# guowentian/dynamicppr

Hardware: AMD Instinct MI355X
Metric: edge-updates/sec (ppr_throughput, summed over sources); ms_per_step = mean per-batch PPR update time (higher is better)
Workload: dtype f64

## Files before the change

### dynamicppr_amd/csrc/dppr_calib.hpp

```cpp
#pragma once

#include "dppr_common.hpp"

namespace dppr {

template <int GB>
__global__ __launch_bounds__(1024) void k_bench_lines(const double2 *__restrict__ table, uint64_t line_mask, int n_per_octet,
                                                      double *__restrict__ sink) {
    const int j = threadIdx.x & 7;
    const uint64_t oct = ((uint64_t)blockIdx.x * 1024 + threadIdx.x) >> 3;
    double a0 = 0.0, a1 = 0.0;
    for (int it = 0; it < n_per_octet; it += GB) {
        double2 v[GB];
#pragma unroll
        for (int k = 0; k < GB; ++k) {
            uint64_t z = oct * (uint64_t)n_per_octet + (uint64_t)(it + k) + 0x9E3779B97F4A7C15ull;
            z = (z ^ (z >> 30)) * 0xBF58476D1CE4E5B9ull;
            z = (z ^ (z >> 27)) * 0x94D049BB133111EBull;
            z ^= z >> 31;
            v[k] = table[(z & line_mask) * 8 + j];
        }
#pragma unroll
        for (int k = 0; k < GB; ++k) {
            a0 += v[k].x;
            a1 += v[k].y;
        }
    }
    if (a0 + a1 == 12345.678) sink[0] = a0;
}

typedef double v2d __attribute__((ext_vector_type(2)));
__global__ __launch_bounds__(1024) void k_bench_copy(const double2 *__restrict__ src2, double2 *__restrict__ dst2, int64_t n16) {
    const v2d *src = reinterpret_cast<const v2d *>(src2);
    v2d *dst = reinterpret_cast<v2d *>(dst2);
    const int64_t stride = (int64_t)gridDim.x * 1024;
    int64_t i = (int64_t)blockIdx.x * 1024 + threadIdx.x;
    for (; i + 3 * stride < n16; i += 4 * stride) {
        const v2d a = src[i], b = src[i + stride];
        const v2d c = src[i + 2 * stride], d = src[i + 3 * stride];
        dst[i] = a;
        dst[i + stride] = b;
        dst[i + 2 * stride] = c;
        dst[i + 3 * stride] = d;
    }
    for (; i < n16; i += stride) dst[i] = src[i];
}

inline int calib_device(int device) {
    int ndev = 0;
    if (hipGetDeviceCount(&ndev) != hipSuccess || device < 0 || device >= ndev) return DPPR_ERR_NO_DEVICE;
    return hipSetDevice(device) == hipSuccess ? DPPR_OK : DPPR_ERR_HIP;
}
template <class Launch>
int time_launches(int reps, float *ms_per_launch, Launch &&launch) {
    hipEvent_t a, b;
    (void)hipEventCreate(&a);
    (void)hipEventCreate(&b);
    launch();
    (void)hipEventRecord(a, 0);
    for (int i = 0; i < reps; ++i) launch();
    (void)hipEventRecord(b, 0);
// ... 11 lines not shown
```

### dynamicppr_amd/csrc/dppr_engine.hip

```cpp
#include <algorithm>
#include <atomic>
#include <cmath>
#include <cstdio>
#include <cstdlib>
#include <cstring>
#include <future>
#include <mutex>
#include <ctime>
#include <string>
#include <type_traits>
#include <unordered_map>
#include <vector>

#include <hip/hip_runtime.h>
#include <rocprim/rocprim.hpp>

#include "../../include/dppr.h"
#include "dppr_churn_plan.hpp"
#include "dppr_cut.hpp"
#include "dppr_devbuf.hpp"
#include "dppr_idspace.hpp"
#include "dppr_loop_plan.hpp"
#include "dppr_query_plan.hpp"
#include "dppr_kernels.hpp"
// ... 1612 lines not shown

int dppr_group_reset_stats(dppr_engine *e, int32_t group) {
    GET_GROUP(e, group);
    HIP_TRY(hipSetDevice(e->device));
    return solve_reset_stats(e, g);
}

int dppr_group_stats(dppr_engine *e, int32_t group, dppr_stats_t *out) {
    GET_GROUP(e, group);
    if (!out) return DPPR_ERR_INVALID;
    HIP_TRY(hipSetDevice(e->device));
    return solve_stats(e, g, out);
}

#ifdef DPPR_STAMPS
extern "C" int dppr_debug_bin_stamps(unsigned long long *out, int which, int rows) {
    return hipMemcpyFromSymbol(out, HIP_SYMBOL(dppr::g_bin_stamps), sizeof(unsigned long long) * 6 * (size_t)rows,
                               sizeof(unsigned long long) * 6 * 16384 * (size_t)which) == hipSuccess ? 0 : -2;
}
extern "C" int dppr_debug_stamps(unsigned long long *out, int rows) {
    return hipMemcpyFromSymbol(out, HIP_SYMBOL(dppr::g_stamps), sizeof(unsigned long long) * 8 * (size_t)rows) == hipSuccess
               ? 0 : -2;
}
#endif

int dppr_bench_atomics(int device, int64_t table_elems, int64_t n, int scope, int reps, float *out_ms) {
    if (table_elems <= 0 || (table_elems & (table_elems - 1)) || n <= 0 || reps <= 0 || !out_ms) return DPPR_ERR_INVALID;
    if (int rc = calib_device(device)) return rc;
    DevBuf<double> table, sink;
    if (table.alloc((size_t)table_elems) != 0) return DPPR_ERR_NOMEM;
    (void)sink.alloc(1);
    (void)hipMemset(table, 0, sizeof(double) * (size_t)table_elems);
    const int grid = 2048;
    return time_launches(reps, out_ms, [&]() {
        if (scope == 2)
            hipLaunchKernelGGL(k_bench_scatter<0>, dim3(grid), dim3(BLOCK), 0, 0, table, (uint64_t)table_elems - 1, n);
        else if (scope == 3)
            hipLaunchKernelGGL(k_bench_scatter<1>, dim3(grid), dim3(BLOCK), 0, 0, table, (uint64_t)table_elems - 1, n);
        else if (scope == 0)
            hipLaunchKernelGGL(k_bench_atomics<__HIP_MEMORY_SCOPE_AGENT>, dim3(grid), dim3(BLOCK), 0, 0, table,
                               (uint64_t)table_elems - 1, n, sink);
        else
            hipLaunchKernelGGL(k_bench_atomics<__HIP_MEMORY_SCOPE_WORKGROUP>, dim3(grid), dim3(BLOCK), 0, 0, table,
                               (uint64_t)table_elems - 1, n, sink);
    });
}

int dppr_bench_line_fills(int device, int64_t table_bytes, int64_t lines, int reps, float *out_ms) {
    if (table_bytes < 128 || (table_bytes & (table_bytes - 1)) || lines <= 0 || reps <= 0 || !out_ms) return DPPR_ERR_INVALID;
    if (int rc = calib_device(device)) return rc;
    DevBuf<double2> table;
    DevBuf<double> sink;
    if (table.alloc((size_t)table_bytes / sizeof(double2)) != 0) return DPPR_ERR_NOMEM;
    (void)sink.alloc(1);
    (void)hipMemset(table, 0, (size_t)table_bytes);
    const int grid = 2048;
    const int per = (int)std::max<int64_t>(8, (lines + (int64_t)grid * 128 - 1) / ((int64_t)grid * 128) / 8 * 8);
    const int rc = time_launches(reps, out_ms, [&]() {
        hipLaunchKernelGGL(k_bench_lines<8>, dim3(grid), dim3(1024), 0, 0, table, (uint64_t)(table_bytes / 128) - 1, per, sink);
    });
    *out_ms = *out_ms * (float)((double)lines / ((double)grid * 128.0 * per));
    return rc;
}

int dppr_bench_stream_copy(int device, int64_t bytes, int reps, float *out_ms) {
    if (bytes < 16 || reps <= 0 || !out_ms) return DPPR_ERR_INVALID;
// ... 51 lines not shown
```

### dynamicppr_amd/csrc/dppr_gpush.hpp

```cpp
#pragma once

#include "dppr_multi.hpp"

namespace dppr {

constexpr int GPUSH_LOG = 16;

struct GPushCtl {
    int n[2];
    int etot;
    int overflow;
    int it;
    int stop;
    unsigned int done;
    int pad;
    int F[GPUSH_LOG][GS_MAX];
    long long atomics[GPUSH_LOG];
};

__global__ __launch_bounds__(BLOCK) void k_gpush_list(const uint32_t *__restrict__ act, int n_words, int *__restrict__ list, int cap,
                                                      GPushCtl *__restrict__ ctl) {
    for (int w = blockIdx.x * BLOCK + threadIdx.x; w < n_words; w += gridDim.x * BLOCK) {
        uint32_t m = act[w];
        if (!m) continue;
        const int n = __popc(m);
        const int pos = atomicAdd(&ctl->n[0], n);
        for (int k = 0; m; ++k, m &= m - 1) {
            if (pos + k < cap) list[pos + k] = w * 32 + (__ffs((int)m) - 1);
            else ctl->overflow = 1;
        }
    }
}

template <int SPL, int GW>
__global__ __launch_bounds__(BLOCK) void k_gpush_rows(const int *__restrict__ list, const GPushCtl *__restrict__ ctl, int which,
                                                      double *__restrict__ x, double *__restrict__ r, bool to_x) {
    if (ctl->overflow) return;
    const int n = ctl->n[which];
    const int j = threadIdx.x & (OCT - 1);
    if (!oct_live<SPL, GW>(j)) return;
    for (int i = (blockIdx.x * BLOCK + threadIdx.x) / OCT; i < n; i += gridDim.x * BLOCK / OCT) {
        const size_t base = (size_t)list[i] * GW + j * SPL, xbase = (size_t)list[i] * x_stride(GW) + j * SPL;
#pragma unroll
        for (int q = 0; q < SPL; ++q) {
            if (to_x) x[xbase + q] = r[base + q];
            else r[base + q] = x[xbase + q];
        }
    }
}

// ... 7 lines not shown
    const int n = ctl->n[which];
    const int *list = which ? list1 : list0;
    if (threadIdx.x < GS_MAX) s_cnt[threadIdx.x] = 0;
    __syncthreads();
    const int j = threadIdx.x & (OCT - 1);
    int nleg[SPL];
#pragma unroll
    for (int q = 0; q < SPL; ++q) nleg[q] = 0;
    const bool live = oct_live<SPL, GW>(j);
    for (int i = (blockIdx.x * BLOCK + threadIdx.x) / OCT; i < n; i += gridDim.x * BLOCK / OCT) {
        const int u = list[i];
        const size_t base = (size_t)u * GW + j * SPL;
#pragma unroll
        for (int q = 0; q < SPL; ++q) {
            if (!live) continue;
            const double rv = r[base + q];
            const bool lg = legal(rv, phase, eps);
            x[(size_t)u * x_stride(GW) + j * SPL + q] = lg ? rv : 0.0;
            if (lg) {
                if (it > 0 || credit_first) p[base + q] = p[base + q] + ALPHA * rv;
                r[base + q] = 0.0;
                nleg[q]++;
            }
        }
        if (j == 0) atomicAnd(&bits[u >> 5], ~(1u << (u & 31)));
    }
#pragma unroll
    for (int q = 0; q < SPL; ++q)
        if (nleg[q]) atomicAdd(&s_cnt[j * SPL + q], nleg[q]);
    __syncthreads();
    if (threadIdx.x < GW && s_cnt[threadIdx.x]) atomicAdd(&ctl->F[it & (GPUSH_LOG - 1)][threadIdx.x], s_cnt[threadIdx.x]);
}

__global__ __launch_bounds__(1024) void k_gpush_scan(GPushCtl *ctl, const int *__restrict__ list0, const int *__restrict__ list1,
                                                     const int *__restrict__ in_row_ptr, int *__restrict__ pre, int max_n,
                                                     long long max_edges) {
    __shared__ long long s_w[16];
    __shared__ long long s_carry;
    if (ctl->stop) return;
    const int which = ctl->it & 1;
    const int n = ctl->n[which];
    const int *list = which ? list1 : list0;
    const int tid = threadIdx.x, lane = lane_id(), w = wave_id();
    if (n > max_n || ctl->overflow) {
        if (tid == 0) ctl->stop = 1;
        return;
    }
    if (tid < GS_MAX) ctl->F[ctl->it & (GPUSH_LOG - 1)][tid] = 0;
    if (tid == 0) ctl->atomics[ctl->it & (GPUSH_LOG - 1)] = 0;
    if (tid == 0) s_carry = 0;
    __syncthreads();
    for (int base = 0; base < n; base += 1024) {
        const int i = base + tid;
        int d = 0;
        if (i < n) {
            const int u = list[i];
            d = in_row_ptr[u + 1] - in_row_ptr[u];
        }
        const int inc = wave_inclusive_scan(d);
        if (lane == WAVE - 1) s_w[w] = inc;
        __syncthreads();
        long long woff = 0;
        for (int k = 0; k < w; ++k) woff += s_w[k];
        const long long carry = s_carry;
        const long long mine = carry + woff + inc - d;
        if (i < n) pre[i] = (int)(mine < 0x7fffffffll ? mine : 0x7fffffffll);
        __syncthreads();
        if (tid == 1023) s_carry = carry + woff + inc;
        __syncthreads();
    }
    if (tid == 0) {
        const long long tot = s_carry;
        if (tot > max_edges || tot > 0x7fffffffll) ctl->stop = 1;
        else {
            pre[n] = (int)tot;
            ctl->etot = (int)tot;
            ctl->n[which ^ 1] = 0;
        }
    }
}

template <int SPL, int GW>
__global__ __launch_bounds__(BLOCK) void k_gpush_expand(const int *__restrict__ list0, const int *__restrict__ list1, GPushCtl *ctl,
                                                        const int *__restrict__ pre, const int *__restrict__ in_row_ptr,
                                                        const Adj *__restrict__ adj, const int *__restrict__ hub_degp1,
                                                        const double *__restrict__ x, double *__restrict__ r,
                                                        uint32_t *__restrict__ bits, int *__restrict__ nlist0, int *__restrict__ nlist1,
                                                        int cap, int phase, double eps, IterStats *__restrict__ stats) {
    __shared__ unsigned long long s_edges;
    if (ctl->stop) return;
    const int it = ctl->it, which = it & 1;
    const int n = ctl->n[which], etot = ctl->etot;
    const int *list = which ? list1 : list0;
    int *nlist = which ? nlist0 : nlist1;
    if (threadIdx.x == 0) s_edges = 0ull;
    __syncthreads();
    const int j = threadIdx.x & (OCT - 1);
    const bool live = oct_live<SPL, GW>(j);
    const long long n_oct = (long long)gridDim.x * (BLOCK / OCT);
    const long long oct = (long long)blockIdx.x * (BLOCK / OCT) + threadIdx.x / OCT;
    const long long per = (etot + n_oct - 1) / n_oct;
    long long e0 = oct * per, e1 = e0 + per < (long long)etot ? e0 + per : (long long)etot;
    unsigned ecount = 0;
    if (e0 < e1 && n > 0) {
        int lo = 0, hi = n;
        while (hi - lo > 1) {
            const int mid = (lo + hi) >> 1;
            if (pre[mid] <= (int)e0) lo = mid; else hi = mid;
        }
        int i = lo;
        while (e0 < e1) {
            while (pre[i + 1] <= (int)e0) ++i;
            const int u = list[i];
            double xv[SPL];
#pragma unroll
            for (int q = 0; q < SPL; ++q) xv[q] = live ? x[(size_t)u * x_stride(GW) + j * SPL + q] : 0.0;
            const long long row_end = pre[i + 1] < (int)e1 ? pre[i + 1] : e1;
            const Adj *row = adj + in_row_ptr[u] + ((int)e0 - pre[i]);
            for (int k = 0; k < (int)(row_end - e0); ++k) {
                const Adj a = row[k];
                const int dp1 = a.degp1 < 0 ? hub_degp1[~a.degp1] : a.degp1;
                const double den = (double)dp1;
                bool crossed = false;
#pragma unroll
                for (int q = 0; q < SPL; ++q) {
                    if (xv[q] != 0.0) {
                        const double add = ONE_MINUS_ALPHA * xv[q] / den;
                        const double prer = atomic_add_ret(&r[(size_t)a.v * GW + j * SPL + q], add);
                        crossed |= !legal(prer, phase, eps) && legal(prer + add, phase, eps);
                        ++ecount;
                    }
                }
                if (oct_mask(__ballot(crossed)) && j == 0) {
                    const uint32_t bit = 1u << (a.v & 31);
                    const uint32_t old = atomicOr(&bits[a.v >> 5], bit);
                    if (!(old & bit)) {
                        const int pos = atomicAdd(&ctl->n[which ^ 1], 1);
                        if (pos < cap) nlist[pos] = a.v;
                        else ctl->overflow = 1;
                    }
                }
            }
            e0 = row_end;
        }
    }
    if (ecount) atomicAdd(&s_edges, (unsigned long long)ecount);
    __syncthreads();
    if (threadIdx.x == 0) {
        if (s_edges) {
            stats->blk_E[blockIdx.x] += s_edges;
            atomicAdd(reinterpret_cast<unsigned long long *>(&ctl->atomics[it & (GPUSH_LOG - 1)]), s_edges);
        }
        __threadfence();
        if (atomicAdd(&ctl->done, 1u) == gridDim.x - 1) {
            ctl->done = 0u;
            if (ctl->n[which ^ 1] > cap) ctl->n[which ^ 1] = cap;
            ctl->it = it + 1;
        }
    }
}

constexpr int TINY_N = 512;
constexpr int TINY_E = 1024;
static_assert(sizeof(double) * TINY_N * 16 + sizeof(int) * (3 * TINY_N + 1) + 1024 <= 160 * 1024,
              "k_gpush_tiny: TINY_N snapshot rows + lists + scan must fit the 160 KB LDS of a gfx950 CU");

template <int SPL, int GW>
__global__ __launch_bounds__(1024) void k_gpush_tiny(GPushCtl *ctl, int *__restrict__ list0, int *__restrict__ list1,
                                                     const int *__restrict__ in_row_ptr, const Adj *__restrict__ adj,
                                                     const int *__restrict__ hub_degp1, double *r, double *p, uint32_t *bits, int phase,
                                                     double eps, IterStats *__restrict__ stats, int max_it, int credit_first) {
    constexpr int NT = 1024, NOCT = NT / OCT;
    __shared__ int s_list[2][TINY_N];
    __shared__ int s_pre[TINY_N + 1];
    __shared__ double s_x[TINY_N * GW];
    __shared__ int s_w[NT / WAVE];
    __shared__ int s_n[2];
    __shared__ int s_cnt[GS_MAX];
    __shared__ int s_flag;
    __shared__ unsigned long long s_edges;
    if (ctl->stop || ctl->overflow) return;
    const int tid = threadIdx.x, lane = lane_id(), w = wave_id();
    const int j = tid & (OCT - 1), oid = tid / OCT;
    const bool live = oct_live<SPL, GW>(j);
    int it = ctl->it, which = it & 1;
    const int n0 = ctl->n[which];
    if (n0 > TINY_N) return;
    for (int i = tid; i < n0; i += NT) s_list[which][i] = (which ? list1 : list0)[i];
    if (tid == 0) {
        s_n[which] = n0;
        s_n[which ^ 1] = 0;
        s_flag = 0;
// ... 21 lines not shown
        if (tid < n) s_pre[tid] = woff + inc - d;
        if (tid == 0) s_pre[n] = tot;
        if (tot > TINY_E) break;
        int nleg[SPL];
#pragma unroll
        for (int q = 0; q < SPL; ++q) nleg[q] = 0;
        for (int i = oid; i < n; i += NOCT) {
            const int u = s_list[which][i];
            const size_t base = (size_t)u * GW + j * SPL;
#pragma unroll
            for (int q = 0; q < SPL; ++q) {
                if (!live) continue;
                double rv = gs_ld<true>(r + base + q);
                const bool lg = legal(rv, phase, eps);
                if (lg) {
                    rv = atomic_exch(r + base + q, 0.0);
                    if (it > 0 || credit_first) (void)__hip_atomic_fetch_add(p + base + q, ALPHA * rv, __ATOMIC_RELAXED, __HIP_MEMORY_SCOPE_AGENT);
                    nleg[q]++;
                }
                s_x[i * GW + j * SPL + q] = lg ? rv : 0.0;
            }
            if (j == 0) (void)atomicAnd(&bits[u >> 5], ~(1u << (u & 31)));
        }
#pragma unroll
        for (int q = 0; q < SPL; ++q)
            if (nleg[q]) atomicAdd(&s_cnt[j * SPL + q], nleg[q]);
        asm volatile("s_waitcnt vmcnt(0)" ::: "memory");
        __syncthreads();
        if (tid < GS_MAX) {
            ctl->F[it & (GPUSH_LOG - 1)][tid] = s_cnt[tid];
            s_cnt[tid] = 0;
        }
        const int e_per = (tot + NOCT - 1) / NOCT;
        int e0 = oid * e_per;
        const int e1 = min(tot, e0 + e_per);
        unsigned long long adds = 0;
        if (e0 < e1) {
            int lo = 0, hi = n;
            while (hi - lo > 1) {
                const int mid = (lo + hi) >> 1;
                if (s_pre[mid] <= e0) lo = mid; else hi = mid;
            }
            int i = lo;
            while (e0 < e1) {
                while (s_pre[i + 1] <= e0) ++i;
                const int u = s_list[which][i];
                double xv[SPL];
#pragma unroll
                for (int q = 0; q < SPL; ++q) xv[q] = live ? s_x[i * GW + j * SPL + q] : 0.0;
                const int row_end = min(s_pre[i + 1], e1);
                const Adj *row = adj + in_row_ptr[u] + (e0 - s_pre[i]);
                for (int k = 0; k < row_end - e0; ++k) {
                    const Adj a = row[k];
                    const double den = (double)(a.degp1 < 0 ? hub_degp1[~a.degp1] : a.degp1);
                    bool crossed = false;
#pragma unroll
                    for (int q = 0; q < SPL; ++q) {
                        if (xv[q] != 0.0) {
                            const double add = ONE_MINUS_ALPHA * xv[q] / den;
                            const double prer = atomic_add_ret(&r[(size_t)a.v * GW + j * SPL + q], add);
                            crossed |= !legal(prer, phase, eps) && legal(prer + add, phase, eps);
                            ++adds;
                        }
                    }
                    if (oct_mask(__ballot(crossed)) && j == 0) {
                        const uint32_t bit = 1u << (a.v & 31);
                        const uint32_t old = atomicOr(&bits[a.v >> 5], bit);
                        if (!(old & bit)) {
                            const int pos = atomicAdd(&s_n[which ^ 1], 1);
                            if (pos < TINY_N) s_list[which ^ 1][pos] = a.v;
                            else s_flag = 1;
                        }
                    }
                }
                e0 = row_end;
            }
        }
        if (adds) atomicAdd(&s_edges, adds);
        __syncthreads();
        if (tid == 0) {
            ctl->atomics[it & (GPUSH_LOG - 1)] = (long long)(s_edges - edges_before);
            edges_before = s_edges;
            s_n[which] = 0;
        }
        ++it;
        which ^= 1;
    }
    __syncthreads();
    const int n = min(s_n[which], TINY_N);
    for (int i = tid; i < n; i += NT) (which ? list1 : list0)[i] = s_list[which][i];
    if (tid == 0) {
        ctl->n[which] = n;
        ctl->n[which ^ 1] = 0;
        ctl->it = it;
        if (s_flag) ctl->stop = 1;
        if (s_edges) stats->blk_E[0] += s_edges;
    }
}

template <int SPL, int GW>
__global__ __launch_bounds__(BLOCK) void k_gpush_leave(int V, const uint32_t *__restrict__ bits, double *__restrict__ x,
                                                       const double *__restrict__ r, double *__restrict__ p, int credit, int phase,
                                                       double eps, int *__restrict__ cnt_out) {
    __shared__ int s_cnt[GS_MAX];
    if (threadIdx.x < GS_MAX) s_cnt[threadIdx.x] = 0;
    __syncthreads();
    const int j = threadIdx.x & (OCT - 1);
    const bool live = oct_live<SPL, GW>(j);
    int nleg[SPL];
#pragma unroll
// ... 23 lines not shown
```

### dynamicppr_amd/csrc/dppr_host_group.hpp

```cpp
#pragma once

namespace {

template <class F>
void with_row(int gw, int nvx, F &&f) {
    auto narrow = [&](auto w) {
        if (nvx == 512) f(IC<1>{}, w, IC<512>{});
        else f(IC<1>{}, w, IC<1024>{});
    };
    switch (gw) {
    case 2: narrow(IC<2>{}); break;
    case 4: narrow(IC<4>{}); break;
    case 6: narrow(IC<6>{}); break;
    case 8: narrow(IC<8>{}); break;
    case 10: f(IC<2>{}, IC<10>{}, IC<512>{}); break;
    case 12: f(IC<2>{}, IC<12>{}, IC<512>{}); break;
    case 14: f(IC<2>{}, IC<14>{}, IC<512>{}); break;
    default: f(IC<2>{}, IC<16>{}, IC<512>{}); break;
    }
}
template <class F>
void with_row(int gw, F &&f) {
    with_row(gw, 512, [&](auto spl, auto w, auto) { f(spl, w); });
}
// ... 36 lines not shown
        cap = std::min(per_cu * cus, STAT_SLOTS);
    }
    return cap;
}

struct PushTail {
    enum How { NOT_ENTERED, CONVERGED, GAVE_BACK } how = NOT_ENTERED;
    int iters = 0;
    bool owed = false;
};

int group_push_tail(dppr_engine *e, Group &g, const Epoch &ep, int phase, double eps, long long pairs_at_entry, PushTail *t) {
    const int cap = std::max(1024, std::min(e->gpush_list_cap, e->V));
    if (g.plist[0].capacity() != (size_t)cap || !g.pctl) {
        HIP_TRY(loop_wait(e));
        g.plist[0].reset(); g.plist[1].reset(); g.ppre.reset(); g.pctl.reset();
        HIP_TRY(g.plist[0].alloc((size_t)cap));
        HIP_TRY(g.plist[1].alloc((size_t)cap));
        HIP_TRY(g.ppre.alloc((size_t)cap + 1));
        HIP_TRY(g.pctl.alloc(1));
    }
    HIP_TRY(hipMemsetAsync(g.pctl, 0, sizeof(GPushCtl), e->stream));
    const int n_words = (ep.grp_n_int + 31) / 32;
    hipLaunchKernelGGL(k_gpush_list, dim3(grid_for(n_words)), dim3(BLOCK), 0, e->stream, g.act[0], n_words, g.plist[0], cap, g.pctl);
    const int rows_grid = grid_for(std::min<long long>(pairs_at_entry, cap), BLOCK / OCT);
    with_row(g.gw, [&](auto spl, auto gw) {
        hipLaunchKernelGGL((k_gpush_rows<decltype(spl)::value, decltype(gw)::value>), dim3(rows_grid), dim3(BLOCK), 0, e->stream, g.plist[0],
                           g.pctl, 0, g.x, g.r, false);
    });
    HIP_TRY(hipGetLastError());
    static thread_local GPushCtl h;
    const int credit_first = t->owed ? 1 : 0;
    const long long max_edges = gpush_edge_bound(e->gpush_max_edges, ep.n_ggroups);
    const int grid = 256;
    static const bool trace = getenv("DPPR_GROUP_TRACE") != nullptr;
    int it_done = 0;
    long long known_n = pairs_at_entry;
    bool tiny_declined = false;
    long long last_adds = gpush_adds_at_entry(pairs_at_entry);
    for (;;) {
        if (gpush_take_tiny(known_n, last_adds, tiny_declined)) {
            with_row(g.gw, [&](auto spl, auto gw) {
                hipLaunchKernelGGL((k_gpush_tiny<decltype(spl)::value, decltype(gw)::value>), dim3(1), dim3(1024), 0, e->stream, g.pctl, g.plist[0],
                                   g.plist[1], ep.row_ptr, ep.adj, ep.hub_degp1, g.r, g.p, g.act[0], phase, eps, g.dstats, GPUSH_LOG, credit_first);
            });
        } else {
        const int m = gpush_chunk(it_done, pairs_at_entry);
        tiny_declined = false;
        for (int k = 0; k < m; ++k) {
            hipLaunchKernelGGL(k_gpush_scan, dim3(1), dim3(1024), 0, e->stream, g.pctl, g.plist[0], g.plist[1], ep.row_ptr, g.ppre, cap - 1, max_edges);
            with_row(g.gw, [&](auto spl, auto gw) {
                constexpr int SPL = decltype(spl)::value, GW = decltype(gw)::value;
                hipLaunchKernelGGL((k_gpush_snap<SPL, GW>), dim3(grid), dim3(BLOCK), 0, e->stream, g.plist[0], g.plist[1], g.pctl, g.x, g.r, g.p,
                                   g.act[0], phase, eps, credit_first);
                hipLaunchKernelGGL((k_gpush_expand<SPL, GW>), dim3(grid), dim3(BLOCK), 0, e->stream, g.plist[0], g.plist[1], g.pctl, g.ppre,
                                   ep.row_ptr, ep.adj, ep.hub_degp1, g.x, g.r, g.act[0], g.plist[0], g.plist[1], cap, phase, eps, g.dstats);
            });
        }
        }
        HIP_TRY(hipGetLastError());
        HIP_TRY(hipMemcpyAsync(&h, g.pctl, sizeof(GPushCtl), hipMemcpyDeviceToHost, e->stream));
        HIP_TRY(loop_wait(e));
        for (int i = it_done; i < h.it; ++i) {
            const long long F = lane_sum(h.F[i & (GPUSH_LOG - 1)]);
            if (F == 0) continue;
            account_iteration(g.st, F, ITER_PUSH);
            ++t->iters;
            if (trace)
                fprintf(stderr, "[gpush ] phase %d iteration +%d  frontier pairs %9lld  adds %lld\n", phase, i, F, h.atomics[i & (GPUSH_LOG - 1)]);
        }
        if (gpush_tiny_declined(h.it > it_done, h.stop != 0, known_n)) tiny_declined = true;
        if (h.it > it_done) last_adds = h.atomics[(h.it - 1) & (GPUSH_LOG - 1)];
        it_done = h.it;
        known_n = h.n[h.it & 1];
        if (h.stop && h.it == 0 && h.overflow) return DPPR_OK;
        if (h.stop) {
            if (trace) fprintf(stderr, "[gpush ] phase %d: an iteration of %d vertices called itself off after %d iterations\n", phase, h.n[h.it & 1], h.it);
            HIP_TRY(hipMemsetAsync(g.cnt, 0, sizeof(int) * 3 * GS_MAX, e->stream));
            with_row(g.gw, [&](auto spl, auto gw) {
                hipLaunchKernelGGL((k_gpush_leave<decltype(spl)::value, decltype(gw)::value>), dim3(grid_for(ep.grp_n_int, BLOCK / OCT)), dim3(BLOCK), 0,
                                   e->stream, ep.grp_n_int, g.act[0], g.x, g.r, g.p, h.it > 0 ? 1 : 0, phase, eps, g.cnt);
            });
            HIP_TRY(hipGetLastError());
            if (h.it > 0) t->owed = false;
            t->how = PushTail::GAVE_BACK;
            return DPPR_OK;
        }
        if (h.n[h.it & 1] == 0) {
            t->how = PushTail::CONVERGED;
            return DPPR_OK;
        }
        if (it_done >= e->max_iters) return fail(e, DPPR_ERR_NOT_CONVERGED, "iteration cap hit");
    }
}

struct GroupLoop {
    dppr_engine *const e;
    Group &g;
    const Epoch &ep;
    const int phase;
    const double eps;
    const int hp = phase == PHASE_BOTH ? 0 : phase;
// ... 183 lines not shown
```

### dynamicppr_amd/csrc/dppr_host_state.hpp

```cpp
#pragma once

static constexpr int CNT_HDR = 16;
static constexpr int PERSIST_RETRY_BATCHES = 64;
static constexpr int GQ_PAD = 32;
static constexpr int BIN_MAX_BLOCKS = 1 << 16, BIN_MAX_BIG = 4096, BIN_SMALL_INTS = BIN_MAX_BLOCKS + BIN_MAX_BIG + 1 + 64;
static constexpr int SU_SPLIT_MIN = 1 << 16;
static constexpr int MERGE_MISS_WORD = 44;

namespace dppr {

inline std::atomic<long long> g_device_bytes{0}, g_pinned_bytes{0};

struct DeviceAlloc {
    static int alloc(void **p, size_t bytes) {
        const hipError_t rc = hipMalloc(p, bytes);
        if (rc == hipSuccess) g_device_bytes.fetch_add((long long)bytes, std::memory_order_relaxed);
        return (int)rc;
    }
    static int free(void *p, size_t bytes) {
        g_device_bytes.fetch_sub((long long)bytes, std::memory_order_relaxed);
        return (int)hipFree(p);
    }
};

// ... 265 lines not shown
    size_t sort_tmp_bytes = 0;
    DevBuf<int> su_grp;
    DevBuf<uint64_t> bk[4];
    DevBuf<uint64_t> bks[4];
    DevBuf<int> delpos;
    struct Pre {
        std::future<bool> task;
        const int32_t *src[4] = {nullptr, nullptr, nullptr, nullptr};
        int n[4] = {0, 0, 0, 0};
        std::vector<int32_t> out[4];
        std::vector<uint32_t> miss[4];
        unsigned long long epoch = 0;
        bool armed = false, ok = false;
    } pre;
    long long pre_hits = 0, pre_misses = 0;
    bool incremental = true;
    bool sweep_bits = false;
    bool hot_blocks = true;
    int gsweep_hot_rows = 24576;
    int gsweep_grid_cap = 0;
    bool group_resident = true;
    int gmulti_cap[2] = {-1, -1};
    bool any_groups = false;
    int ggroups_min = 256;
    bool force_radix_grouping = false;
    bool cost_model = true;
    bool group_full_rows = false;
    bool wide_groups = false;
    bool group_tail_seeding = true;
    int gpush_enter_pairs = -1;
    int gpush_list_cap = 1 << 20;
    long long gpush_max_edges = 0;
    int gpush_auto_factor = 2;
    int bin_mode = 1;
    int bin_ha_tiles = 128, bin_hb_tiles = 60;
    long long bin_target = 0;
    long long bin_target_a = 4ll << 20;
    long long bin_min_ids = 1ll << 19;
    DevBuf<int> bin_vblk_a;
    DevBuf<unsigned long long> bin_scan;
    DevBuf<int> bin_small;
    long long bin_chunk = 32768;
    DevBuf<double> bin_vals;
    DevBuf<uint64_t> bin_wb, bin_wa;
    DevBuf<int> bin_first;
    std::vector<int32_t> bin_cut_a, bin_cut_b;
    int bin_abits = 0, bin_bbits = 0;
    int bin_cut_ids = 0;
    bool bin_words_valid = false;
    int bin_slides_since_cut = 0;
    bool bin_incremental = true;
    int bin_recut_every = 32;
    bool bin_frozen_rebuild = false;
    bool bin_force_full = false;
    int bin_miss_host = 0;
    long long bin_patched = 0, bin_rebuilt = 0;
    DevBuf<unsigned char> bin_tmp;
    size_t bin_tmp_bytes = 0;
    bool bin_ready = false;
    std::vector<int32_t> h_tiles_in;
    DevBuf<uint32_t> su_k[2], su_v[2];
    DevBuf<double> su_term;
    DevBuf<uint8_t> su_ins;
    DevBuf<unsigned char> su_tmp;
    size_t su_tmp_bytes = 0;
    std::vector<int32_t> st_b1, st_b2;
// ... 178 lines not shown
```

Baseline: 54.67 million.

## Fuse gpush scan into expand, batch edges per octet, size grid from occupancy

The per-iteration scan kernel launch is folded into the tail of the expand kernel: the last block to finish rescans the next frontier, so only the first scan is launched separately. Edge expansion now processes K edges per octet in lockstep, with lanes loading adjacency in parallel and atomics issued back to back. New-frontier appends go through a block-level shared buffer to cut global atomics, and the expand grid is sized from occupancy and the edge bound rather than a fixed 256 blocks. This adds a cross-block completion protocol with relaxed atomics and more register pressure, and it includes a row-atomics benchmark plus trace timing.

Result: no change. 54.52 million (median of 3 runs) (-0.3%).

```diff
diff --git a/dynamicppr_amd/csrc/dppr_calib.hpp b/dynamicppr_amd/csrc/dppr_calib.hpp
--- a/dynamicppr_amd/csrc/dppr_calib.hpp
+++ b/dynamicppr_amd/csrc/dppr_calib.hpp
@@ -27,6 +27,33 @@
         }
     }
     if (a0 + a1 == 12345.678) sink[0] = a0;
+}
+
+template <int KF, int SPL>
+__global__ __launch_bounds__(BLOCK) void k_bench_row_atomics(double *table, uint64_t n_rows, int row_doubles, int lanes, int n_per_octet,
+                                                             double *__restrict__ sink) {
+    const int j = threadIdx.x & 7;
+    const uint64_t oct = ((uint64_t)blockIdx.x * BLOCK + threadIdx.x) >> 3;
+    double acc = 0.0;
+    for (int it = 0; it < n_per_octet; it += KF) {
+        double ret[KF][SPL];
+#pragma unroll
+        for (int k = 0; k < KF; ++k) {
+            uint64_t z = oct * (uint64_t)n_per_octet + (uint64_t)(it + k) + 0x9E3779B97F4A7C15ull;
+            z = (z ^ (z >> 30)) * 0xBF58476D1CE4E5B9ull;
+            z = (z ^ (z >> 27)) * 0x94D049BB133111EBull;
+            z ^= z >> 31;
+            const uint64_t row = ((z >> 32) * n_rows) >> 32;
+#pragma unroll
+            for (int q = 0; q < SPL; ++q)
+                ret[k][q] = j < lanes ? atomic_add_ret(&table[row * (uint64_t)row_doubles + j * SPL + q], 1e-9) : 0.0;
+        }
+#pragma unroll
+        for (int k = 0; k < KF; ++k)
+#pragma unroll
+            for (int q = 0; q < SPL; ++q) acc += ret[k][q];
+    }
+    if (acc == 12345.678) sink[0] = acc;
 }
 
 typedef double v2d __attribute__((ext_vector_type(2)));
diff --git a/dynamicppr_amd/csrc/dppr_engine.hip b/dynamicppr_amd/csrc/dppr_engine.hip
--- a/dynamicppr_amd/csrc/dppr_engine.hip
+++ b/dynamicppr_amd/csrc/dppr_engine.hip
@@ -1668,6 +1668,25 @@
     (void)sink.alloc(1);
     (void)hipMemset(table, 0, sizeof(double) * (size_t)table_elems);
     const int grid = 2048;
+    if (scope >= 16) {
+        const int kc = (scope - 16) / 4, wc = (scope - 16) % 4;
+        if (kc > 2 || wc > 2 || n > (int64_t)1 << 40) return DPPR_ERR_INVALID;
+        const int row_doubles = wc == 0 ? 8 : wc == 1 ? 10 : 16, lanes = wc == 1 ? 5 : 8;
+        const uint64_t n_rows = (uint64_t)table_elems / row_doubles;
+        const int64_t octs = (int64_t)grid * (BLOCK / 8);
+        const int per = (int)std::min<int64_t>(1 << 20, std::max<int64_t>(8, (n + octs - 1) / octs / 8 * 8));
+        if (n_rows < 1 || n_rows > 0xffffffffull) return DPPR_ERR_INVALID;
+        const int rc = time_launches(reps, out_ms, [&]() {
+            auto go = [&](auto kf, auto spl) {
+                hipLaunchKernelGGL((k_bench_row_atomics<decltype(kf)::value, decltype(spl)::value>), dim3(grid), dim3(BLOCK), 0, 0, table, n_rows,
+                                   row_doubles, lanes, per, sink);
+            };
+            auto width = [&](auto kf) { wc == 0 ? go(kf, IC<1>{}) : go(kf, IC<2>{}); };
+            kc == 0 ? width(IC<1>{}) : kc == 1 ? width(IC<4>{}) : width(IC<8>{});
+        });
+        *out_ms = *out_ms * (float)((double)n / ((double)octs * per));
+        return rc;
+    }
     return time_launches(reps, out_ms, [&]() {
         if (scope == 2)
             hipLaunchKernelGGL(k_bench_scatter<0>, dim3(grid), dim3(BLOCK), 0, 0, table, (uint64_t)table_elems - 1, n);
diff --git a/dynamicppr_amd/csrc/dppr_gpush.hpp b/dynamicppr_amd/csrc/dppr_gpush.hpp
--- a/dynamicppr_amd/csrc/dppr_gpush.hpp
+++ b/dynamicppr_amd/csrc/dppr_gpush.hpp
@@ -8,14 +8,14 @@
 
 struct GPushCtl {
     int n[2];
-    int etot;
-    int overflow;
+    int etot[2];
     int it;
     int stop;
     unsigned int done;
-    int pad;
+    int overflow;
     int F[GPUSH_LOG][GS_MAX];
     long long atomics[GPUSH_LOG];
+    int edges[GPUSH_LOG];
 };
 
 __global__ __launch_bounds__(BLOCK) void k_gpush_list(const uint32_t *__restrict__ act, int n_words, int *__restrict__ list, int cap,
@@ -89,41 +89,49 @@
     if (threadIdx.x < GW && s_cnt[threadIdx.x]) atomicAdd(&ctl->F[it & (GPUSH_LOG - 1)][threadIdx.x], s_cnt[threadIdx.x]);
 }
 
-__global__ __launch_bounds__(1024) void k_gpush_scan(GPushCtl *ctl, const int *__restrict__ list0, const int *__restrict__ list1,
-                                                     const int *__restrict__ in_row_ptr, int *__restrict__ pre, int max_n,
-                                                     long long max_edges) {
-    __shared__ long long s_w[16];
+__device__ __forceinline__ int gpush_ld(const int *p) { return __hip_atomic_load(p, __ATOMIC_RELAXED, __HIP_MEMORY_SCOPE_AGENT); }
+__device__ __forceinline__ void gpush_st(int *p, int v) { __hip_atomic_store(p, v, __ATOMIC_RELAXED, __HIP_MEMORY_SCOPE_AGENT); }
+
+constexpr int SCAN_ITEMS = 4;
+template <int NT>
+__device__ __forceinline__ void gpush_scan_list(GPushCtl *ctl, const int *list, int n, int which, int it, bool overflow,
+                                                const int *__restrict__ in_row_ptr, int *__restrict__ pre, int max_n, long long max_edges) {
+    __shared__ long long s_w[NT / WAVE];
     __shared__ long long s_carry;
-    if (ctl->stop) return;
-    const int which = ctl->it & 1;
-    const int n = ctl->n[which];
-    const int *list = which ? list1 : list0;
     const int tid = threadIdx.x, lane = lane_id(), w = wave_id();
-    if (n > max_n || ctl->overflow) {
+    if (n > max_n || overflow) {
         if (tid == 0) ctl->stop = 1;
         return;
     }
-    if (tid < GS_MAX) ctl->F[ctl->it & (GPUSH_LOG - 1)][tid] = 0;
-    if (tid == 0) ctl->atomics[ctl->it & (GPUSH_LOG - 1)] = 0;
+    if (tid < GS_MAX) ctl->F[it & (GPUSH_LOG - 1)][tid] = 0;
+    if (tid == 0) ctl->atomics[it & (GPUSH_LOG - 1)] = 0;
     if (tid == 0) s_carry = 0;
     __syncthreads();
-    for (int base = 0; base < n; base += 1024) {
-        const int i = base + tid;
-        int d = 0;
-        if (i < n) {
-            const int u = list[i];
-            d = in_row_ptr[u + 1] - in_row_ptr[u];
-        }
-        const int inc = wave_inclusive_scan(d);
+    for (int base = 0; base < n; base += NT * SCAN_ITEMS) {
+        const int i0 = base + tid * SCAN_ITEMS;
+        int u[SCAN_ITEMS], d[SCAN_ITEMS];
+#pragma unroll
+        for (int q = 0; q < SCAN_ITEMS; ++q) u[q] = i0 + q < n ? gpush_ld(list + i0 + q) : -1;
+        int sum = 0;
+#pragma unroll
+        for (int q = 0; q < SCAN_ITEMS; ++q) {
+            d[q] = u[q] >= 0 ? in_row_ptr[u[q] + 1] - in_row_ptr[u[q]] : 0;
+            sum += d[q];
+        }
+        const int inc = wave_inclusive_scan(sum);
         if (lane == WAVE - 1) s_w[w] = inc;
         __syncthreads();
         long long woff = 0;
         for (int k = 0; k < w; ++k) woff += s_w[k];
         const long long carry = s_carry;
-        const long long mine = carry + woff + inc - d;
-        if (i < n) pre[i] = (int)(mine < 0x7fffffffll ? mine : 0x7fffffffll);
-        __syncthreads();
-        if (tid == 1023) s_carry = carry + woff + inc;
+        long long mine = carry + woff + inc - sum;
+#pragma unroll
+        for (int q = 0; q < SCAN_ITEMS; ++q) {
+            if (i0 + q < n) pre[i0 + q] = (int)(mine < 0x7fffffffll ? mine : 0x7fffffffll);
+            mine += d[q];
+        }
+        __syncthreads();
+        if (tid == NT - 1) s_carry = carry + woff + inc;
         __syncthreads();
     }
     if (tid == 0) {
@@ -131,77 +139,161 @@
         if (tot > max_edges || tot > 0x7fffffffll) ctl->stop = 1;
         else {
             pre[n] = (int)tot;
-            ctl->etot = (int)tot;
+            ctl->etot[it & 1] = (int)tot;
+            ctl->edges[it & (GPUSH_LOG - 1)] = (int)tot;
             ctl->n[which ^ 1] = 0;
         }
     }
 }
 
-template <int SPL, int GW>
-__global__ __launch_bounds__(BLOCK) void k_gpush_expand(const int *__restrict__ list0, const int *__restrict__ list1, GPushCtl *ctl,
-                                                        const int *__restrict__ pre, const int *__restrict__ in_row_ptr,
-                                                        const Adj *__restrict__ adj, const int *__restrict__ hub_degp1,
-                                                        const double *__restrict__ x, double *__restrict__ r,
-                                                        uint32_t *__restrict__ bits, int *__restrict__ nlist0, int *__restrict__ nlist1,
-                                                        int cap, int phase, double eps, IterStats *__restrict__ stats) {
-    __shared__ unsigned long long s_edges;
+__global__ __launch_bounds__(1024) void k_gpush_scan(GPushCtl *ctl, const int *list0, const int *list1, const int *__restrict__ in_row_ptr,
+                                                     int *__restrict__ pre, int max_n, long long max_edges) {
     if (ctl->stop) return;
     const int it = ctl->it, which = it & 1;
-    const int n = ctl->n[which], etot = ctl->etot;
+    gpush_scan_list<1024>(ctl, which ? list1 : list0, ctl->n[which], which, it, ctl->overflow != 0, in_row_ptr, pre, max_n, max_edges);
+}
+
+constexpr int GPUSH_K = 4;
+constexpr int GPUSH_APP = 512;
+constexpr int GPUSH_SHARE = 2 * GPUSH_K;
+
+__device__ __forceinline__ int gpush_active_blocks(int etot, int grid) {
+    constexpr int PER_BLOCK = GPUSH_SHARE * (BLOCK / OCT);
+    const long long want = ((long long)etot + PER_BLOCK - 1) / PER_BLOCK;
+    return (int)(want < 1 ? 1 : want < grid ? want : grid);
+}
+
+template <int SPL, int GW, typename XRow, typename Queue>
+__device__ __forceinline__ unsigned gpush_expand_share(int e0, int e1, int n, const int *pre, const int *list,
+                                                       const int *__restrict__ in_row_ptr, const Adj *__restrict__ adj,
+                                                       const int *__restrict__ hub_degp1, double *r, uint32_t *bits, int phase, double eps,
+                                                       XRow xrow, Queue queue) {
+    constexpr int K = GPUSH_K;
+    static_assert(K <= OCT, "a lane per edge of a batch");
+    if (e0 >= e1 || n <= 0) return 0u;
+    const int j = threadIdx.x & (OCT - 1);
+    const int lane0 = lane_id() & ~(OCT - 1);
+    const bool live = oct_live<SPL, GW>(j);
+    unsigned adds = 0;
+    int lo = 0, hi = n;
+    while (hi - lo > 1) {
+        const int span = hi - lo;
+        const int held = __popc(oct_mask(__ballot(pre[lo + span * (j + 1) / (OCT + 1)] <= e0)));
+        if (held < OCT) hi = lo + span * (held + 1) / (OCT + 1);
+        if (held > 0) lo = lo + span * held / (OCT + 1);
+    }
+    int i = lo;
+    for (int b = e0; b < e1; b += K) {
+        const int nb = e1 - b < K ? e1 - b : K;
+        int ii = i, uu = 0, av = 0, dp1 = 1;
+        if (j < nb) {
+            const int e = b + j;
+            while (pre[ii + 1] <= e) ++ii;
+            uu = list[ii];
+            const Adj a = adj[in_row_ptr[uu] + (e - pre[ii])];
+            av = a.v;
+            dp1 = a.degp1 < 0 ? hub_degp1[~a.degp1] : a.degp1;
+        }
+        i = __shfl(ii, lane0 + nb - 1);
+        int vk[K];
+        double add[K][SPL], prer[K][SPL];
+        unsigned act = 0;
+#pragma unroll
+        for (int k = 0; k < K; ++k) {
+            vk[k] = __shfl(av, lane0 + k);
+            const double den = (double)__shfl(dp1, lane0 + k);
+            const int ik = __shfl(ii, lane0 + k), uk = __shfl(uu, lane0 + k);
+#pragma unroll
+            for (int q = 0; q < SPL; ++q) {
+                const double xv = (k < nb && live) ? xrow(ik, uk)[j * SPL + q] : 0.0;
+                add[k][q] = ONE_MINUS_ALPHA * xv / den;
+                prer[k][q] = 0.0;
+                if (xv != 0.0) act |= 1u << (k * SPL + q);
+            }
+        }
+#pragma unroll
+        for (int k = 0; k < K; ++k)
+#pragma unroll
+            for (int q = 0; q < SPL; ++q)
+                if (act & (1u << (k * SPL + q))) prer[k][q] = atomic_add_ret(&r[(size_t)vk[k] * GW + j * SPL + q], add[k][q]);
+        adds += __popc(act);
+        bool queue_mine = false;
+#pragma unroll
+        for (int k = 0; k < K; ++k) {
+            bool crossed = false;
+#pragma unroll
+            for (int q = 0; q < SPL; ++q)
+                if (act & (1u << (k * SPL + q))) crossed |= !legal(prer[k][q], phase, eps) && legal(prer[k][q] + add[k][q], phase, eps);
+            if (oct_mask(__ballot(crossed)) && j == k) queue_mine = true;
+        }
+        bool append = false;
+        if (queue_mine) {
+            const uint32_t bit = 1u << (av & 31);
+            append = !(atomicOr(&bits[av >> 5], bit) & bit);
+        }
+        const uint64_t am = __ballot(append);
+        if (am) {
+            const int leader = __ffsll((unsigned long long)am) - 1;
+            int pos = 0;
+            if (lane_id() == leader) pos = queue.reserve(__popcll(am));
+            pos = __shfl(pos, leader) + mbcnt(am);
+            if (append) queue.put(pos, av);
+        }
+    }
+    return adds;
+}
+
+template <int SPL, int GW>
+__global__ __launch_bounds__(BLOCK) void k_gpush_expand(int *list0, int *list1, GPushCtl *ctl, int *pre, const int *__restrict__ in_row_ptr,
+                                                        const Adj *__restrict__ adj, const int *__restrict__ hub_degp1,
+                                                        const double *__restrict__ x, double *r, uint32_t *bits, int cap, int phase, double eps,
+                                                        IterStats *__restrict__ stats, int max_n, long long max_edges, int it) {
+    constexpr int K = GPUSH_K;
+    __shared__ unsigned long long s_edges;
+    __shared__ int s_close;
+    __shared__ int s_app[GPUSH_APP], s_napp, s_base;
+    if (ctl->stop) return;
+    const int which = it & 1;
+    const int etot = ctl->etot[which];
+    const int n_act = gpush_active_blocks(etot, (int)gridDim.x);
+    if ((int)blockIdx.x >= n_act) return;
+    const int n = ctl->n[which];
     const int *list = which ? list1 : list0;
-    int *nlist = which ? nlist0 : nlist1;
-    if (threadIdx.x == 0) s_edges = 0ull;
-    __syncthreads();
-    const int j = threadIdx.x & (OCT - 1);
-    const bool live = oct_live<SPL, GW>(j);
-    const long long n_oct = (long long)gridDim.x * (BLOCK / OCT);
+    int *nlist = which ? list0 : list1;
+    if (threadIdx.x == 0) {
+        s_edges = 0ull;
+        s_napp = 0;
+    }
+    __syncthreads();
+    const long long n_oct = (long long)n_act * (BLOCK / OCT);
     const long long oct = (long long)blockIdx.x * (BLOCK / OCT) + threadIdx.x / OCT;
-    const long long per = (etot + n_oct - 1) / n_oct;
-    long long e0 = oct * per, e1 = e0 + per < (long long)etot ? e0 + per : (long long)etot;
+    const long long per = ((etot + n_oct - 1) / n_oct + K - 1) / K * K;
+    const long long e0 = oct * per, e1 = e0 + per < (long long)etot ? e0 + per : (long long)etot;
+    struct {
+        GPushCtl *ctl;
+        int *nlist, *app, *napp;
+        int which, cap;
+        __device__ int reserve(int cnt) const { return atomicAdd(napp, cnt); }
+        __device__ void put(int pos, int v) const {
+            if (pos < GPUSH_APP) app[pos] = v;
+            else put_global(atomicAdd(&ctl->n[which ^ 1], 1), v);
+        }
+        __device__ void put_global(int pos, int v) const {
+            if (pos < cap) gpush_st(nlist + pos, v);
+            else atomicOr(&ctl->overflow, 1);
+        }
+    } queue{ctl, nlist, s_app, &s_napp, which, cap};
     unsigned ecount = 0;
-    if (e0 < e1 && n > 0) {
-        int lo = 0, hi = n;
-        while (hi - lo > 1) {
-            const int mid = (lo + hi) >> 1;
-            if (pre[mid] <= (int)e0) lo = mid; else hi = mid;
-        }
-        int i = lo;
-        while (e0 < e1) {
-            while (pre[i + 1] <= (int)e0) ++i;
-            const int u = list[i];
-            double xv[SPL];
-#pragma unroll
-            for (int q = 0; q < SPL; ++q) xv[q] = live ? x[(size_t)u * x_stride(GW) + j * SPL + q] : 0.0;
-            const long long row_end = pre[i + 1] < (int)e1 ? pre[i + 1] : e1;
-            const Adj *row = adj + in_row_ptr[u] + ((int)e0 - pre[i]);
-            for (int k = 0; k < (int)(row_end - e0); ++k) {
-                const Adj a = row[k];
-                const int dp1 = a.degp1 < 0 ? hub_degp1[~a.degp1] : a.degp1;
-                const double den = (double)dp1;
-                bool crossed = false;
-#pragma unroll
-                for (int q = 0; q < SPL; ++q) {
-                    if (xv[q] != 0.0) {
-                        const double add = ONE_MINUS_ALPHA * xv[q] / den;
-                        const double prer = atomic_add_ret(&r[(size_t)a.v * GW + j * SPL + q], add);
-                        crossed |= !legal(prer, phase, eps) && legal(prer + add, phase, eps);
-                        ++ecount;
-                    }
-                }
-                if (oct_mask(__ballot(crossed)) && j == 0) {
-                    const uint32_t bit = 1u << (a.v & 31);
-                    const uint32_t old = atomicOr(&bits[a.v >> 5], bit);
-                    if (!(old & bit)) {
-                        const int pos = atomicAdd(&ctl->n[which ^ 1], 1);
-                        if (pos < cap) nlist[pos] = a.v;
-                        else ctl->overflow = 1;
-                    }
-                }
-            }
-            e0 = row_end;
-        }
-    }
+    if (e0 < e1)
+        ecount = gpush_expand_share<SPL, GW>((int)e0, (int)e1, n, pre, list, in_row_ptr, adj, hub_degp1, r, bits, phase, eps,
+                                             [&](int, int u) { return x + (size_t)u * x_stride(GW); }, queue);
     if (ecount) atomicAdd(&s_edges, (unsigned long long)ecount);
+    __syncthreads();
+    const int napp = s_napp < GPUSH_APP ? s_napp : GPUSH_APP;
+    if (threadIdx.x == 0 && napp) s_base = atomicAdd(&ctl->n[which ^ 1], napp);
+    __syncthreads();
+    for (int a = threadIdx.x; a < napp; a += BLOCK) queue.put_global(s_base + a, s_app[a]);
+    asm volatile("s_waitcnt vmcnt(0)" ::: "memory");
     __syncthreads();
     if (threadIdx.x == 0) {
         if (s_edges) {
@@ -209,12 +301,23 @@
             atomicAdd(reinterpret_cast<unsigned long long *>(&ctl->atomics[it & (GPUSH_LOG - 1)]), s_edges);
         }
         __threadfence();
-        if (atomicAdd(&ctl->done, 1u) == gridDim.x - 1) {
-            ctl->done = 0u;
-            if (ctl->n[which ^ 1] > cap) ctl->n[which ^ 1] = cap;
-            ctl->it = it + 1;
-        }
-    }
+        asm volatile("s_waitcnt vmcnt(0)" ::: "memory");
+        const bool last = atomicAdd(&ctl->done, 1u) == (unsigned)n_act - 1u;
+        if (last) __builtin_amdgcn_fence(__ATOMIC_ACQUIRE, "agent");
+        s_close = last ? 1 : 0;
+    }
+    __syncthreads();
+    if (!s_close) return;
+    int n1 = gpush_ld(&ctl->n[which ^ 1]);
+    const bool overflow = gpush_ld(&ctl->overflow) != 0;
+    if (n1 > cap) n1 = cap;
+    if (threadIdx.x == 0) {
+        ctl->done = 0u;
+        ctl->n[which ^ 1] = n1;
+        ctl->it = it + 1;
+    }
+    __syncthreads();
+    gpush_scan_list<BLOCK>(ctl, nlist, n1, which ^ 1, it + 1, overflow, in_row_ptr, pre, max_n, max_edges);
 }
 
 constexpr int TINY_N = 512;
@@ -302,50 +405,19 @@
             s_cnt[tid] = 0;
         }
         const int e_per = (tot + NOCT - 1) / NOCT;
-        int e0 = oid * e_per;
+        const int e0 = oid * e_per;
         const int e1 = min(tot, e0 + e_per);
-        unsigned long long adds = 0;
-        if (e0 < e1) {
-            int lo = 0, hi = n;
-            while (hi - lo > 1) {
-                const int mid = (lo + hi) >> 1;
-                if (s_pre[mid] <= e0) lo = mid; else hi = mid;
+        struct {
+            int *cnt, *nlist, *flag;
+            __device__ int reserve(int c) const { return atomicAdd(cnt, c); }
+            __device__ void put(int pos, int v) const {
+                if (pos < TINY_N) nlist[pos] = v;
+                else *flag = 1;
             }
-            int i = lo;
-            while (e0 < e1) {
-                while (s_pre[i + 1] <= e0) ++i;
-                const int u = s_list[which][i];
-                double xv[SPL];
-#pragma unroll
-                for (int q = 0; q < SPL; ++q) xv[q] = live ? s_x[i * GW + j * SPL + q] : 0.0;
-                const int row_end = min(s_pre[i + 1], e1);
-                const Adj *row = adj + in_row_ptr[u] + (e0 - s_pre[i]);
-                for (int k = 0; k < row_end - e0; ++k) {
-                    const Adj a = row[k];
-                    const double den = (double)(a.degp1 < 0 ? hub_degp1[~a.degp1] : a.degp1);
-                    bool crossed = false;
-#pragma unroll
-                    for (int q = 0; q < SPL; ++q) {
-                        if (xv[q] != 0.0) {
-                            const double add = ONE_MINUS_ALPHA * xv[q] / den;
-                            const double prer = atomic_add_ret(&r[(size_t)a.v * GW + j * SPL + q], add);
-                            crossed |= !legal(prer, phase, eps) && legal(prer + add, phase, eps);
-                            ++adds;
-                        }
-                    }
-                    if (oct_mask(__ballot(crossed)) && j == 0) {
-                        const uint32_t bit = 1u << (a.v & 31);
-                        const uint32_t old = atomicOr(&bits[a.v >> 5], bit);
-                        if (!(old & bit)) {
-                            const int pos = atomicAdd(&s_n[which ^ 1], 1);
-                            if (pos < TINY_N) s_list[which ^ 1][pos] = a.v;
-                            else s_flag = 1;
-                        }
-                    }
-                }
-                e0 = row_end;
-            }
-        }
+        } queue{&s_n[which ^ 1], s_list[which ^ 1], &s_flag};
+        const double *sx = s_x;
+        const unsigned long long adds = gpush_expand_share<SPL, GW>(e0, e1, n, s_pre, s_list[which], in_row_ptr, adj, hub_degp1, r, bits, phase,
+                                                                    eps, [&](int i, int) { return sx + i * GW; }, queue);
         if (adds) atomicAdd(&s_edges, adds);
         __syncthreads();
         if (tid == 0) {
diff --git a/dynamicppr_amd/csrc/dppr_host_group.hpp b/dynamicppr_amd/csrc/dppr_host_group.hpp
--- a/dynamicppr_amd/csrc/dppr_host_group.hpp
+++ b/dynamicppr_amd/csrc/dppr_host_group.hpp
@@ -92,8 +92,19 @@
     static thread_local GPushCtl h;
     const int credit_first = t->owed ? 1 : 0;
     const long long max_edges = gpush_edge_bound(e->gpush_max_edges, ep.n_ggroups);
-    const int grid = 256;
+    if (e->gpush_grid_cap <= 0) {
+        int per_cu = 0, cus = 0;
+        if (hipOccupancyMaxActiveBlocksPerMultiprocessor(&per_cu, k_gpush_expand<2, 16>, BLOCK, 0) != hipSuccess || per_cu <= 0) per_cu = 8;
+        if (hipDeviceGetAttribute(&cus, hipDeviceAttributeMultiprocessorCount, e->device) != hipSuccess || cus <= 0) cus = 256;
+        e->gpush_grid_cap = std::min(per_cu * cus, STAT_SLOTS);
+    }
+    const int edges_per_block = GPUSH_SHARE * (BLOCK / OCT);
+    const int grid = (int)std::max<long long>(1, std::min<long long>(e->gpush_grid_cap, (max_edges + edges_per_block - 1) / edges_per_block));
+    const int snap_grid = std::max(256, std::min(grid, 1024));
     static const bool trace = getenv("DPPR_GROUP_TRACE") != nullptr;
+    bool scanned = false;
+    const bool timed = trace && e->profiling;
+    int n_timed = 0;
     int it_done = 0;
     long long known_n = pairs_at_entry;
     bool tiny_declined = false;
@@ -104,19 +115,28 @@
                 hipLaunchKernelGGL((k_gpush_tiny<decltype(spl)::value, decltype(gw)::value>), dim3(1), dim3(1024), 0, e->stream, g.pctl, g.plist[0],
                                    g.plist[1], ep.row_ptr, ep.adj, ep.hub_degp1, g.r, g.p, g.act[0], phase, eps, g.dstats, GPUSH_LOG, credit_first);
             });
+            scanned = false;
+            n_timed = 0;
         } else {
-        const int m = gpush_chunk(it_done, pairs_at_entry);
+        const int m = std::min(gpush_chunk(it_done, pairs_at_entry), GPUSH_LOG - 1);
         tiny_declined = false;
+        if (!scanned)
+            hipLaunchKernelGGL(k_gpush_scan, dim3(1), dim3(1024), 0, e->stream, g.pctl, g.plist[0], g.plist[1], ep.row_ptr, g.ppre, cap - 1, max_edges);
         for (int k = 0; k < m; ++k) {
-            hipLaunchKernelGGL(k_gpush_scan, dim3(1), dim3(1024), 0, e->stream, g.pctl, g.plist[0], g.plist[1], ep.row_ptr, g.ppre, cap - 1, max_edges);
+            int rc = DPPR_OK;
             with_row(g.gw, [&](auto spl, auto gw) {
                 constexpr int SPL = decltype(spl)::value, GW = decltype(gw)::value;
-                hipLaunchKernelGGL((k_gpush_snap<SPL, GW>), dim3(grid), dim3(BLOCK), 0, e->stream, g.plist[0], g.plist[1], g.pctl, g.x, g.r, g.p,
+                hipLaunchKernelGGL((k_gpush_snap<SPL, GW>), dim3(snap_grid), dim3(BLOCK), 0, e->stream, g.plist[0], g.plist[1], g.pctl, g.x, g.r, g.p,
                                    g.act[0], phase, eps, credit_first);
-                hipLaunchKernelGGL((k_gpush_expand<SPL, GW>), dim3(grid), dim3(BLOCK), 0, e->stream, g.plist[0], g.plist[1], g.pctl, g.ppre,
-                                   ep.row_ptr, ep.adj, ep.hub_degp1, g.x, g.r, g.act[0], g.plist[0], g.plist[1], cap, phase, eps, g.dstats);
-            });
-        }
+                rc = timed_launch(e, k, timed, [&] {
+                    hipLaunchKernelGGL((k_gpush_expand<SPL, GW>), dim3(grid), dim3(BLOCK), 0, e->stream, g.plist[0], g.plist[1], g.pctl, g.ppre,
+                                       ep.row_ptr, ep.adj, ep.hub_degp1, g.x, g.r, g.act[0], cap, phase, eps, g.dstats, cap - 1, max_edges, it_done + k);
+                });
+            });
+            if (rc) return rc;
+        }
+        scanned = true;
+        n_timed = timed ? m : 0;
         }
         HIP_TRY(hipGetLastError());
         HIP_TRY(hipMemcpyAsync(&h, g.pctl, sizeof(GPushCtl), hipMemcpyDeviceToHost, e->stream));
@@ -126,8 +146,12 @@
             if (F == 0) continue;
             account_iteration(g.st, F, ITER_PUSH);
             ++t->iters;
-            if (trace)
-                fprintf(stderr, "[gpush ] phase %d iteration +%d  frontier pairs %9lld  adds %lld\n", phase, i, F, h.atomics[i & (GPUSH_LOG - 1)]);
+            if (trace) {
+                float ms = -1e-3f;
+                if (i - it_done < n_timed) HIP_TRY(hipEventElapsedTime(&ms, e->evpool[2 * (i - it_done)], e->evpool[2 * (i - it_done) + 1]));
+                fprintf(stderr, "[gpush ] phase %d iteration +%d  frontier pairs %9lld  adds %lld  expand %.1f us  in-edges %d\n", phase, i, F,
+                        h.atomics[i & (GPUSH_LOG - 1)], ms * 1e3, i - it_done < n_timed ? h.edges[i & (GPUSH_LOG - 1)] : -1);
+            }
         }
         if (gpush_tiny_declined(h.it > it_done, h.stop != 0, known_n)) tiny_declined = true;
         if (h.it > it_done) last_adds = h.atomics[(h.it - 1) & (GPUSH_LOG - 1)];
diff --git a/dynamicppr_amd/csrc/dppr_host_state.hpp b/dynamicppr_amd/csrc/dppr_host_state.hpp
--- a/dynamicppr_amd/csrc/dppr_host_state.hpp
+++ b/dynamicppr_amd/csrc/dppr_host_state.hpp
@@ -321,6 +321,7 @@
     int gpush_list_cap = 1 << 20;
     long long gpush_max_edges = 0;
     int gpush_auto_factor = 2;
+    int gpush_grid_cap = 0;
     int bin_mode = 1;
     int bin_ha_tiles = 128, bin_hb_tiles = 60;
     long long bin_target = 0;
```
